# facebook/winterfell

Measured on NVIDIA H100. Metric: prover_ms, lower is better.
Workload: dtype u64

## Files before the change

### winterfell_b200/csrc/gl64.cuh

```cuda
#pragma once
#ifdef __CUDACC_RTC__
typedef unsigned long long uint64_t;
typedef unsigned int uint32_t;
typedef unsigned char uint8_t;
#else
#include <stdint.h>
#endif

#ifdef __CUDACC__
#define GL_HD __host__ __device__ __forceinline__
#else
#define GL_HD inline
#endif

typedef uint64_t u64;
typedef uint32_t u32;
typedef uint8_t u8;

#define GL_P 0xffffffff00000001ULL
#define GL_EPS 0xffffffffULL
#define GL_GENERATOR 7ULL
#define GL_TWO_ADIC_ROOT 7277203076849721926ULL

static inline u64 gl_add_host(u64 a, u64 b) {
    u64 r = a + b;
    if (r < a || r >= GL_P) r += GL_EPS;
    return r;
}
static inline u64 gl_sub_host(u64 a, u64 b) {
    u64 r = a - b;
    if (a < b) r -= GL_EPS;
    return r;
}
static inline u64 gl_reduce128_host(u64 lo, u64 hi) {
    u64 hh = hi >> 32, hl = hi & GL_EPS;
    u64 t = lo - hh;
    if (lo < hh) t -= GL_EPS;
    u64 m = (hl << 32) - hl;
    u64 r = t + m;
    if (r < m) r += GL_EPS;
    if (r >= GL_P) r -= GL_P;
    return r;
}

#if defined(__CUDACC__) && !defined(GL_LITERAL_EPS)
static __constant__ u32 GL_EPS_CONST = 0xffffffffu;
#define GL_EPS_OPERAND , "r"(GL_EPS_CONST)
#define GL_EPSM(n) "%" #n
#else
#define GL_EPS_OPERAND
#define GL_EPSM(n) "0xffffffff"
#endif
#ifdef __CUDA_ARCH__
__device__ __forceinline__ u64 gl_sub(u64 a, u64 b) {
    u64 r;
    asm("{\n\t"
        ".reg .u32 a0, a1, b0, b1, m;\n\t"
        "mov.b64 {a0, a1}, %1;\n\t"
        "mov.b64 {b0, b1}, %2;\n\t"
        "sub.cc.u32 a0, a0, b0;\n\t"
        "subc.cc.u32 a1, a1, b1;\n\t"
        "subc.u32 m, 0, 0;\n\t"
        "sub.cc.u32 a0, a0, m;\n\t"
        "subc.u32 a1, a1, 0;\n\t"
        "mov.b64 %0, {a0, a1};\n\t"
        "}"
        : "=l"(r)
        : "l"(a), "l"(b));
    return r;
}
__device__ __forceinline__ u64 gl_add(u64 a, u64 b) {
    u64 r;
    asm("{\n\t"
        ".reg .u32 a0, a1, b0, b1, m;\n\t"
        "mov.b64 {a0, a1}, %1;\n\t"
        "mov.b64 {b0, b1}, %2;\n\t"
        "sub.cc.u32 b0, 1, b0;\n\t"
        "subc.u32 b1, 0xffffffff, b1;\n\t"
        "sub.cc.u32 a0, a0, b0;\n\t"
        "subc.cc.u32 a1, a1, b1;\n\t"
        "subc.u32 m, 0, 0;\n\t"
        "sub.cc.u32 a0, a0, m;\n\t"
        "subc.u32 a1, a1, 0;\n\t"
        "mov.b64 %0, {a0, a1};\n\t"
        "}"
        : "=l"(r)
        : "l"(a), "l"(b));
    return r;
}
__device__ __forceinline__ void gl_butterfly(u64& a, u64& b) {
    u64 s, d;
    asm("{\n\t"
        ".reg .u32 a0, a1, b0, b1, n0, n1, s0, s1, m;\n\t"
        "mov.b64 {a0, a1}, %2;\n\t"
        "mov.b64 {b0, b1}, %3;\n\t"
        "sub.cc.u32 n0, 1, b0;\n\t"
        "subc.u32 n1, 0xffffffff, b1;\n\t"
        "sub.cc.u32 s0, a0, n0;\n\t"
        "subc.cc.u32 s1, a1, n1;\n\t"
        "subc.u32 m, 0, 0;\n\t"
        "sub.cc.u32 s0, s0, m;\n\t"
        "subc.u32 s1, s1, 0;\n\t"
        "mov.b64 %0, {s0, s1};\n\t"
        "sub.cc.u32 a0, a0, b0;\n\t"
        "subc.cc.u32 a1, a1, b1;\n\t"
        "subc.u32 m, 0, 0;\n\t"
        "sub.cc.u32 a0, a0, m;\n\t"
        "subc.u32 a1, a1, 0;\n\t"
        "mov.b64 %1, {a0, a1};\n\t"
        "}"
        : "=l"(s), "=l"(d)
        : "l"(a), "l"(b));
    a = s;
    b = d;
}
__device__ __forceinline__ u64 gl_canon(u64 r) {
    u64 o;
    asm("{\n\t"
        ".reg .u32 r0, r1, t0, t1, k;\n\t"
        "mov.b64 {r0, r1}, %1;\n\t"
        "add.cc.u32 t0, r0, 0xffffffff;\n\t"
        "addc.cc.u32 t1, r1, 0;\n\t"
        "addc.u32 k, 0, 0;\n\t"
        "sub.u32 r0, r0, k;\n\t"
        "add.u32 r1, r1, k;\n\t"
        "mov.b64 %0, {r0, r1};\n\t"
        "}"
        : "=l"(o)
        : "l"(r));
    return o;
}
__device__ __forceinline__ u64 gl_reduce128(u64 lo, u64 hi) {
    u64 r;
    asm("{\n\t"
        ".reg .u32 c0, c1, c2, c3, k, m, t0, t1;\n\t"
        "mov.b64 {c0, c1}, %1;\n\t"
        "mov.b64 {c2, c3}, %2;\n\t"
        "sub.cc.u32 c0, c0, c3;\n\t"
        "subc.cc.u32 c1, c1, 0;\n\t"
        "subc.u32 m, 0, 0;\n\t"
        "sub.cc.u32 c0, c0, m;\n\t"
        "subc.u32 c1, c1, 0;\n\t"
        "mad.lo.cc.u32 c0, c2, " GL_EPSM(3) ", c0;\n\t"
        "madc.hi.cc.u32 c1, c2, " GL_EPSM(3) ", c1;\n\t"
        "addc.u32 k, 0, 0;\n\t"
        "add.cc.u32 t0, c0, 0xffffffff;\n\t"
        "addc.cc.u32 t1, c1, 0;\n\t"
        "addc.u32 k, k, 0;\n\t"
        "mad.lo.cc.u32 c0, k, " GL_EPSM(3) ", c0;\n\t"
        "madc.hi.u32 c1, k, " GL_EPSM(3) ", c1;\n\t"
        "mov.b64 %0, {c0, c1};\n\t"
        "}"
        : "=l"(r)
        : "l"(lo), "l"(hi) GL_EPS_OPERAND);
    return r;
}
__device__ __forceinline__ u64 gl_mul(u64 a, u64 b) {
    u64 r;
    asm("{\n\t"
        ".reg .u32 a0, a1, b0, b1, c0, c1, c2, c3, o0, o1, o2, k, m, t0, t1;\n\t"
        "mov.b64 {a0, a1}, %1;\n\t"
        "mov.b64 {b0, b1}, %2;\n\t"
        "mul.lo.u32 c0, a0, b0;\n\t"
        "mul.hi.u32 c1, a0, b0;\n\t"
        "mul.lo.u32 c2, a1, b1;\n\t"
        "mul.hi.u32 c3, a1, b1;\n\t"
        "mul.lo.u32 o0, a0, b1;\n\t"
        "mul.hi.u32 o1, a0, b1;\n\t"
        "mad.lo.cc.u32 o0, a1, b0, o0;\n\t"
        "madc.hi.cc.u32 o1, a1, b0, o1;\n\t"
        "addc.u32 o2, 0, 0;\n\t"
        "add.cc.u32 c1, c1, o0;\n\t"
        "addc.cc.u32 c2, c2, o1;\n\t"
        "addc.u32 c3, c3, o2;\n\t"
        "sub.cc.u32 c0, c0, c3;\n\t"
        "subc.cc.u32 c1, c1, 0;\n\t"
        "subc.u32 m, 0, 0;\n\t"
        "sub.cc.u32 c0, c0, m;\n\t"
        "subc.u32 c1, c1, 0;\n\t"
        "mad.lo.cc.u32 c0, c2, " GL_EPSM(3) ", c0;\n\t"
        "madc.hi.cc.u32 c1, c2, " GL_EPSM(3) ", c1;\n\t"
        "addc.u32 k, 0, 0;\n\t"
        "add.cc.u32 t0, c0, 0xffffffff;\n\t"
        "addc.cc.u32 t1, c1, 0;\n\t"
        "addc.u32 k, k, 0;\n\t"
        "mad.lo.cc.u32 c0, k, " GL_EPSM(3) ", c0;\n\t"
        "madc.hi.u32 c1, k, " GL_EPSM(3) ", c1;\n\t"
        "mov.b64 %0, {c0, c1};\n\t"
        "}"
        : "=l"(r)
        : "l"(a), "l"(b) GL_EPS_OPERAND);
    return r;
}
__device__ __forceinline__ u64 gl_mul_weak(u64 a, u64 b) {
    u64 r;
    asm("{\n\t"
        ".reg .u32 a0, a1, b0, b1, c0, c1, c2, c3, o0, o1, o2, k, m;\n\t"
        "mov.b64 {a0, a1}, %1;\n\t"
        "mov.b64 {b0, b1}, %2;\n\t"
        "mul.lo.u32 c0, a0, b0;\n\t"
        "mul.hi.u32 c1, a0, b0;\n\t"
        "mul.lo.u32 c2, a1, b1;\n\t"
        "mul.hi.u32 c3, a1, b1;\n\t"
        "mul.lo.u32 o0, a0, b1;\n\t"
        "mul.hi.u32 o1, a0, b1;\n\t"
        "mad.lo.cc.u32 o0, a1, b0, o0;\n\t"
        "madc.hi.cc.u32 o1, a1, b0, o1;\n\t"
        "addc.u32 o2, 0, 0;\n\t"
        "add.cc.u32 c1, c1, o0;\n\t"
        "addc.cc.u32 c2, c2, o1;\n\t"
        "addc.u32 c3, c3, o2;\n\t"
        "sub.cc.u32 c0, c0, c3;\n\t"
        "subc.cc.u32 c1, c1, 0;\n\t"
        "subc.u32 m, 0, 0;\n\t"
        "sub.cc.u32 c0, c0, m;\n\t"
        "subc.u32 c1, c1, 0;\n\t"
        "mad.lo.cc.u32 c0, c2, " GL_EPSM(3) ", c0;\n\t"
        "madc.hi.cc.u32 c1, c2, " GL_EPSM(3) ", c1;\n\t"
        "addc.u32 k, 0, 0;\n\t"
        "mad.lo.cc.u32 c0, k, " GL_EPSM(3) ", c0;\n\t"
        "madc.hi.u32 c1, k, " GL_EPSM(3) ", c1;\n\t"
        "mov.b64 %0, {c0, c1};\n\t"
        "}"
        : "=l"(r)
        : "l"(a), "l"(b) GL_EPS_OPERAND);
    return r;
}
__device__ __forceinline__ u64 gl_sqr_weak(u64 a) {
    u64 r;
    asm("{\n\t"
        ".reg .u32 a0, a1, c0, c1, c2, c3, o0, o1, o2, k, m;\n\t"
        ".reg .u64 w;\n\t"
        "mov.b64 {a0, a1}, %1;\n\t"
        "mul.wide.u32 w, a0, a0;\n\t"
        "mov.b64 {c0, c1}, w;\n\t"
        "mul.wide.u32 w, a1, a1;\n\t"
        "mov.b64 {c2, c3}, w;\n\t"
        "mul.wide.u32 w, a0, a1;\n\t"
        "mov.b64 {o0, o1}, w;\n\t"
        "add.cc.u32 o0, o0, o0;\n\t"
        "addc.cc.u32 o1, o1, o1;\n\t"
        "addc.u32 o2, 0, 0;\n\t"
        "add.cc.u32 c1, c1, o0;\n\t"
        "addc.cc.u32 c2, c2, o1;\n\t"
        "addc.u32 c3, c3, o2;\n\t"
        "sub.cc.u32 c0, c0, c3;\n\t"
        "subc.cc.u32 c1, c1, 0;\n\t"
        "subc.u32 m, 0, 0;\n\t"
        "sub.cc.u32 c0, c0, m;\n\t"
        "subc.u32 c1, c1, 0;\n\t"
        "mad.lo.cc.u32 c0, c2, " GL_EPSM(2) ", c0;\n\t"
        "madc.hi.cc.u32 c1, c2, " GL_EPSM(2) ", c1;\n\t"
        "addc.u32 k, 0, 0;\n\t"
        "mad.lo.cc.u32 c0, k, " GL_EPSM(2) ", c0;\n\t"
        "madc.hi.u32 c1, k, " GL_EPSM(2) ", c1;\n\t"
        "mov.b64 %0, {c0, c1};\n\t"
        "}"
        : "=l"(r)
        : "l"(a) GL_EPS_OPERAND);
    return r;
}
template <int K>
__device__ __forceinline__ u64 gl_shl_dev(u64 x) {
    constexpr int R = K & 31;
    const u32 x0 = (u32)x, x1 = (u32)(x >> 32);
    const u32 y0 = x0 << R, y1 = R ? __funnelshift_l(x0, x1, R) : x1, y2 = R ? (x1 >> ((32 - R) & 31)) : 0;
    u64 o;
    if (K < 32) {
        asm("{\n\t"
            ".reg .u32 r0, r1, k, t0, t1;\n\t"
            "mad.lo.cc.u32 r0, %3, " GL_EPSM(4) ", %1;\n\t"
            "madc.hi.cc.u32 r1, %3, " GL_EPSM(4) ", %2;\n\t"
            "addc.u32 k, 0, 0;\n\t"
            "add.cc.u32 t0, r0, 0xffffffff;\n\t"
            "addc.cc.u32 t1, r1, 0;\n\t"
            "addc.u32 k, k, 0;\n\t"
            "mad.lo.cc.u32 r0, k, " GL_EPSM(4) ", r0;\n\t"
            "madc.hi.u32 r1, k, " GL_EPSM(4) ", r1;\n\t"
            "mov.b64 %0, {r0, r1};\n\t"
            "}" : "=l"(o) : "r"(y0), "r"(y1), "r"(y2) GL_EPS_OPERAND);
    } else if (K < 64) {
        asm("{\n\t"
            ".reg .u32 r0, r1, k, m, t0, t1;\n\t"
            "sub.cc.u32 r0, 0, %3;\n\t"
            "subc.cc.u32 r1, %1, 0;\n\t"
            "subc.u32 m, 0, 0;\n\t"
            "sub.cc.u32 r0, r0, m;\n\t"
            "subc.u32 r1, r1, 0;\n\t"
            "mad.lo.cc.u32 r0, %2, " GL_EPSM(4) ", r0;\n\t"
            "madc.hi.cc.u32 r1, %2, " GL_EPSM(4) ", r1;\n\t"
            "addc.u32 k, 0, 0;\n\t"
            "add.cc.u32 t0, r0, 0xffffffff;\n\t"
            "addc.cc.u32 t1, r1, 0;\n\t"
            "addc.u32 k, k, 0;\n\t"
            "mad.lo.cc.u32 r0, k, " GL_EPSM(4) ", r0;\n\t"
            "madc.hi.u32 r1, k, " GL_EPSM(4) ", r1;\n\t"
            "mov.b64 %0, {r0, r1};\n\t"
            "}" : "=l"(o) : "r"(y0), "r"(y1), "r"(y2) GL_EPS_OPERAND);
    } else {
        asm("{\n\t"
            ".reg .u32 m0, m1, b;\n\t"
            "mul.lo.u32 m0, %1, " GL_EPSM(4) ";\n\t"
            "mul.hi.u32 m1, %1, " GL_EPSM(4) ";\n\t"
            "sub.cc.u32 m0, m0, %2;\n\t"
            "subc.cc.u32 m1, m1, %3;\n\t"
            "subc.u32 b, 0, 0;\n\t"
            "sub.cc.u32 m0, m0, b;\n\t"
            "subc.u32 m1, m1, 0;\n\t"
            "mov.b64 %0, {m0, m1};\n\t"
            "}" : "=l"(o) : "r"(y0), "r"(y1), "r"(y2) GL_EPS_OPERAND);
    }
    return o;
}
#else
GL_HD u64 gl_add(u64 a, u64 b) { return gl_add_host(a, b); }
GL_HD u64 gl_sub(u64 a, u64 b) { return gl_sub_host(a, b); }
GL_HD u64 gl_reduce128(u64 lo, u64 hi) { return gl_reduce128_host(lo, hi); }
GL_HD u64 gl_mul(u64 a, u64 b) {
    unsigned __int128 x = (unsigned __int128)a * b;
    return gl_reduce128((u64)x, (u64)(x >> 64));
}
GL_HD u64 gl_mul_weak(u64 a, u64 b) { return gl_mul(a, b); }
GL_HD u64 gl_sqr_weak(u64 a) { return gl_mul(a, a); }
static inline void gl_butterfly(u64& a, u64& b) {
    u64 s = gl_add(a, b);
    b = gl_sub(a, b);
    a = s;
}
#endif
#ifdef __CUDACC__
struct GlAcc {
    u32 w0, w1, w2, w3, w4;
};
__device__ __forceinline__ GlAcc acc_zero() { return GlAcc{0, 0, 0, 0, 0}; }
__device__ __forceinline__ void acc_mad(GlAcc& a, u64 x, u64 y) {
    asm("{\n\t"
        ".reg .u32 x0, x1, y0, y1, m0, m1, m2;\n\t"
        "mov.b64 {x0, x1}, %5;\n\t"
        "mov.b64 {y0, y1}, %6;\n\t"
        "mul.lo.u32 m0, x0, y1;\n\t"
        "mul.hi.u32 m1, x0, y1;\n\t"
        "mad.lo.cc.u32 m0, x1, y0, m0;\n\t"
        "madc.hi.cc.u32 m1, x1, y0, m1;\n\t"
        "addc.u32 m2, 0, 0;\n\t"
        "mad.lo.cc.u32 %0, x0, y0, %0;\n\t"
        "madc.hi.cc.u32 %1, x0, y0, %1;\n\t"
        "madc.lo.cc.u32 %2, x1, y1, %2;\n\t"
        "madc.hi.cc.u32 %3, x1, y1, %3;\n\t"
        "addc.u32 %4, %4, 0;\n\t"
        "add.cc.u32 %1, %1, m0;\n\t"
        "addc.cc.u32 %2, %2, m1;\n\t"
        "addc.cc.u32 %3, %3, m2;\n\t"
        "addc.u32 %4, %4, 0;\n\t"
        "}"
        : "+r"(a.w0), "+r"(a.w1), "+r"(a.w2), "+r"(a.w3), "+r"(a.w4)
        : "l"(x), "l"(y));
}
__device__ __forceinline__ u64 acc_reduce(const GlAcc& a) {
    const u64 t = gl_reduce128((u64)a.w0 | ((u64)a.w1 << 32), (u64)a.w2 | ((u64)a.w3 << 32));
    return gl_sub(t, (u64)a.w4 << 32);
}
#endif
GL_HD u64 gl_neg(u64 a) { return a ? GL_P - a : 0; }
GL_HD u64 gl_dbl(u64 a) { return gl_add(a, a); }
GL_HD u64 gl_sqr(u64 a) { return gl_mul(a, a); }

template <int K>
GL_HD u64 gl_mul_2exp(u64 x) {
    if (K == 0) return x;
    if (K == 96) return gl_neg(x);
#ifdef __CUDA_ARCH__
    return gl_shl_dev<K>(x);
#else
    if (K < 64) return gl_reduce128(x << (K & 63), x >> ((64 - K) & 63));
    u64 yl = x << ((K - 64) & 63), yh = (K == 64) ? 0 : (x >> ((128 - K) & 63));
    u64 r = gl_reduce128(0, yl);
    return gl_sub(r, gl_reduce128(yh << 32, 0));
#endif
}

GL_HD u64 gl_pow(u64 a, u64 e) {
    u64 r = 1;
    while (e) {
        if (e & 1) r = gl_mul(r, a);
        a = gl_mul(a, a);
        e >>= 1;
    }
    return r;
}
GL_HD u64 gl_sqr_n(u64 a, int n) {
    for (int i = 0; i < n; i++) a = gl_sqr(a);
    return a;
}
GL_HD u64 gl_inv(u64 x) {
    u64 e2 = gl_mul(gl_sqr(x), x);
    u64 e4 = gl_mul(gl_sqr_n(e2, 2), e2);
    u64 e8 = gl_mul(gl_sqr_n(e4, 4), e4);
    u64 e16 = gl_mul(gl_sqr_n(e8, 8), e8);
    u64 e24 = gl_mul(gl_sqr_n(e16, 8), e8);
    u64 e28 = gl_mul(gl_sqr_n(e24, 4), e4);
    u64 e30 = gl_mul(gl_sqr_n(e28, 2), e2);
    u64 e31 = gl_mul(gl_sqr(e30), x);
    u64 a2 = gl_sqr(e31);
    u64 b = gl_mul(a2, x);
    return gl_mul(gl_sqr_n(a2, 32), b);
}
GL_HD u64 gl_root_of_unity(u32 log_n) { return gl_pow(GL_TWO_ADIC_ROOT, 1ULL << (32 - log_n)); }
GL_HD u64 gl_from_mont(u64 m) { return gl_mul(m, 18446744065119617025ULL); }
GL_HD u64 gl_to_mont(u64 x) { return gl_mul(x, GL_EPS); }

template <int D>
struct GlExt {
    u64 v[D];
};

template <int D>
GL_HD GlExt<D> ext_zero() {
    GlExt<D> r;
#pragma unroll
    for (int i = 0; i < D; i++) r.v[i] = 0;
    return r;
}
template <int D>
GL_HD GlExt<D> ext_from_base(u64 b) {
    GlExt<D> r = ext_zero<D>();
    r.v[0] = b;
    return r;
}
template <int D>
GL_HD GlExt<D> ext_add(const GlExt<D>& a, const GlExt<D>& b) {
    GlExt<D> r;
#pragma unroll
    for (int i = 0; i < D; i++) r.v[i] = gl_add(a.v[i], b.v[i]);
    return r;
}
template <int D>
GL_HD GlExt<D> ext_sub(const GlExt<D>& a, const GlExt<D>& b) {
    GlExt<D> r;
#pragma unroll
    for (int i = 0; i < D; i++) r.v[i] = gl_sub(a.v[i], b.v[i]);
    return r;
}
template <int D>
GL_HD GlExt<D> ext_mul_base(const GlExt<D>& a, u64 b) {
    GlExt<D> r;
#pragma unroll
    for (int i = 0; i < D; i++) r.v[i] = gl_mul(a.v[i], b);
    return r;
}
GL_HD GlExt<1> ext_mul(const GlExt<1>& a, const GlExt<1>& b) {
    GlExt<1> r;
    r.v[0] = gl_mul(a.v[0], b.v[0]);
    return r;
}
GL_HD GlExt<2> ext_mul(const GlExt<2>& a, const GlExt<2>& b) {
    GlExt<2> r;
    u64 a0b0 = gl_mul(a.v[0], b.v[0]);
    r.v[0] = gl_sub(a0b0, gl_dbl(gl_mul(a.v[1], b.v[1])));
    r.v[1] = gl_sub(gl_mul(gl_add(a.v[0], a.v[1]), gl_add(b.v[0], b.v[1])), a0b0);
    return r;
}
GL_HD GlExt<3> ext_mul(const GlExt<3>& a, const GlExt<3>& b) {
    GlExt<3> r;
    u64 a0b0 = gl_mul(a.v[0], b.v[0]), a1b1 = gl_mul(a.v[1], b.v[1]), a2b2 = gl_mul(a.v[2], b.v[2]);
    u64 s01 = gl_mul(gl_add(a.v[0], a.v[1]), gl_add(b.v[0], b.v[1]));
    u64 s02 = gl_mul(gl_add(a.v[0], a.v[2]), gl_add(b.v[0], b.v[2]));
    u64 s12 = gl_mul(gl_add(a.v[1], a.v[2]), gl_add(b.v[1], b.v[2]));
    u64 m = gl_sub(a0b0, a1b1);
    r.v[0] = gl_sub(gl_add(s12, m), a2b2);
    r.v[1] = gl_sub(gl_sub(gl_add(s01, s12), gl_dbl(a1b1)), a0b0);
    r.v[2] = gl_sub(s02, m);
    return r;
}
GL_HD GlExt<1> ext_frobenius(const GlExt<1>& x) { return x; }
GL_HD GlExt<2> ext_frobenius(const GlExt<2>& x) {
    GlExt<2> r;
    r.v[0] = gl_add(x.v[0], x.v[1]);
    r.v[1] = gl_neg(x.v[1]);
    return r;
}
GL_HD GlExt<3> ext_frobenius(const GlExt<3>& x) {
    GlExt<3> r;
    r.v[0] = gl_add(x.v[0], gl_add(gl_mul(10615703402128488253ULL, x.v[1]), gl_mul(6700183068485440220ULL, x.v[2])));
    r.v[1] = gl_add(gl_mul(10050274602728160328ULL, x.v[1]), gl_mul(14531223735771536287ULL, x.v[2]));
    r.v[2] = gl_add(gl_mul(11746561000929144102ULL, x.v[1]), gl_mul(8396469466686423992ULL, x.v[2]));
    return r;
}
GL_HD GlExt<1> ext_inv(const GlExt<1>& a) {
    GlExt<1> r;
    r.v[0] = gl_inv(a.v[0]);
    return r;
}
GL_HD GlExt<2> ext_inv(const GlExt<2>& a) {
    if ((a.v[0] | a.v[1]) == 0) return a;
    GlExt<2> num = ext_frobenius(a);
    GlExt<2> norm = ext_mul(a, num);
    return ext_mul_base(num, gl_inv(norm.v[0]));
}
GL_HD GlExt<3> ext_inv(const GlExt<3>& a) {
    if ((a.v[0] | a.v[1] | a.v[2]) == 0) return a;
    GlExt<3> c1 = ext_frobenius(a);
    GlExt<3> c2 = ext_frobenius(c1);
    GlExt<3> num = ext_mul(c1, c2);
    GlExt<3> norm = ext_mul(a, num);
    return ext_mul_base(num, gl_inv(norm.v[0]));
}
template <int D>
GL_HD GlExt<D> ext_pow(GlExt<D> a, u64 e) {
    GlExt<D> r = ext_from_base<D>(1);
    while (e) {
        if (e & 1) r = ext_mul(r, a);
        a = ext_mul(a, a);
        e >>= 1;
    }
    return r;
}
```

### winterfell_b200/csrc/minidft.cuh

```cuda
#pragma once
#include "gl64.cuh"

__device__ __forceinline__ void bf2(u64& a, u64& b) { gl_butterfly(a, b); }
template <int R>
__device__ __forceinline__ void mini_dft(u64* x);
template <>
__device__ __forceinline__ void mini_dft<1>(u64* x) { bf2(x[0], x[1]); }
template <>
__device__ __forceinline__ void mini_dft<2>(u64* x) {
    bf2(x[0], x[2]);
    bf2(x[1], x[3]);
    x[3] = gl_mul_2exp<48>(x[3]);
    bf2(x[0], x[1]);
    bf2(x[2], x[3]);
}
template <>
__device__ __forceinline__ void mini_dft<3>(u64* x);
template <>
__device__ __forceinline__ void mini_dft<3>(u64* x) {
    bf2(x[0], x[4]);
    bf2(x[1], x[5]);
    bf2(x[2], x[6]);
    bf2(x[3], x[7]);
    x[5] = gl_mul_2exp<24>(x[5]);
    x[6] = gl_mul_2exp<48>(x[6]);
    x[7] = gl_mul_2exp<72>(x[7]);
    mini_dft<2>(x);
    mini_dft<2>(x + 4);
}
template <>
__device__ __forceinline__ void mini_dft<4>(u64* x) {
    bf2(x[0], x[8]);
    bf2(x[1], x[9]);
    bf2(x[2], x[10]);
    bf2(x[3], x[11]);
    bf2(x[4], x[12]);
    bf2(x[5], x[13]);
    bf2(x[6], x[14]);
    bf2(x[7], x[15]);
    x[9] = gl_mul_2exp<12>(x[9]);
    x[10] = gl_mul_2exp<24>(x[10]);
    x[11] = gl_mul_2exp<36>(x[11]);
    x[12] = gl_mul_2exp<48>(x[12]);
    x[13] = gl_mul_2exp<60>(x[13]);
    x[14] = gl_mul_2exp<72>(x[14]);
    x[15] = gl_mul_2exp<84>(x[15]);
    mini_dft<3>(x);
    mini_dft<3>(x + 8);
}
template <>
__device__ __forceinline__ void mini_dft<5>(u64* x) {
#pragma unroll
    for (int q = 0; q < 16; q++) bf2(x[q], x[q + 16]);
    x[17] = gl_mul_2exp<6>(x[17]);
    x[18] = gl_mul_2exp<12>(x[18]);
    x[19] = gl_mul_2exp<18>(x[19]);
    x[20] = gl_mul_2exp<24>(x[20]);
    x[21] = gl_mul_2exp<30>(x[21]);
    x[22] = gl_mul_2exp<36>(x[22]);
    x[23] = gl_mul_2exp<42>(x[23]);
    x[24] = gl_mul_2exp<48>(x[24]);
    x[25] = gl_mul_2exp<54>(x[25]);
    x[26] = gl_mul_2exp<60>(x[26]);
    x[27] = gl_mul_2exp<66>(x[27]);
    x[28] = gl_mul_2exp<72>(x[28]);
    x[29] = gl_mul_2exp<78>(x[29]);
    x[30] = gl_mul_2exp<84>(x[30]);
    x[31] = gl_mul_2exp<90>(x[31]);
    mini_dft<4>(x);
    mini_dft<4>(x + 16);
}
__device__ __forceinline__ u32 brev(u32 v, int bits) { return __brev(v) >> (32 - bits); }

__device__ __forceinline__ u64 tw_lookup(const u64* tab, u32 e, u32 half) {
    u64 t = tab[e & (half - 1)];
    return (e & half) ? gl_neg(t) : t;
}
```

### winterfell_b200/csrc/ntt2.cu

```cuda
#include "minidft.cuh"
#include "ntt.cuh"

#ifndef NTT2_THREADS
#define NTT2_THREADS 256
#endif
#ifndef NTT2_MINB
#define NTT2_MINB 2
#endif
#define NTT2_TILE_ELEMS 8192

template <int LOGS>
struct Plan {
    static constexpr int rounds = LOGS >= 9 ? 3 : 2;
    static constexpr int r0 = (LOGS == 8) ? 4 : 3;
    static constexpr int r1 = (LOGS == 11 || LOGS == 8 || LOGS == 7) ? 4 : 3;
    static constexpr int r2 = LOGS >= 9 ? LOGS - r0 - r1 : 0;
    static_assert(LOGS >= 6 && LOGS <= 11, "plan covers 2^6 .. 2^11");
    static_assert(r0 + r1 + r2 == LOGS && (rounds == 2 || (r2 == 3 || r2 == 4)), "radices must add up");
    static constexpr int lanes = LOGS == 11 ? 4 : 8;
    static constexpr int tw0_entries = 1 << LOGS;
    static constexpr int tw1_entries = rounds == 3 ? (1 << (LOGS - r0)) : 0;
    static constexpr int tw_entries = tw0_entries + tw1_entries;
};
template <int LOGS> __host__ __device__ constexpr int plan_radix(int k) { return k == 0 ? Plan<LOGS>::r0 : (k == 1 ? Plan<LOGS>::r1 : Plan<LOGS>::r2); }
template <int LOGS> __host__ __device__ constexpr int plan_stage(int k) { return k == 0 ? 0 : (k == 1 ? Plan<LOGS>::r0 : Plan<LOGS>::r0 + Plan<LOGS>::r1); }

template <int LK>
__host__ __device__ constexpr u32 swz_const(u32 r) {
    u32 x = r >> LK, h = 0;
    while (x) { h ^= x & ((1u << LK) - 1); x >>= LK; }
    return h;
}
template <int LK>
__device__ __forceinline__ u32 swz_hash(u32 r) {
    if (LK == 1) return __popc(r >> 1) & 1;
    u32 x = r >> 2;
    x ^= x >> 4;
    x ^= x >> 8;
    x ^= x >> 2;
    return x & 3;
}
template <int LK>
__device__ __forceinline__ u32 prow(u32 r) { return r ^ swz_hash<LK>(r); }

__device__ __forceinline__ void bulk_init(u64* mbar, int tid) {
    if (tid == 0) {
        u32 mb = (u32)__cvta_generic_to_shared(mbar);
        asm volatile("mbarrier.init.shared::cta.b64 [%0], 1;" ::"r"(mb));
        asm volatile("fence.mbarrier_init.release.cluster;" ::: "memory");
    }
}
__device__ __forceinline__ void bulk_expect(u64* mbar, u32 bytes) {
    u32 mb = (u32)__cvta_generic_to_shared(mbar);
    asm volatile("mbarrier.arrive.expect_tx.shared::cta.b64 _, [%0], %1;" ::"r"(mb), "r"(bytes) : "memory");
}
__device__ __forceinline__ void bulk_copy(void* smem_dst, const void* gsrc, u32 bytes, u64* mbar) {
    u32 mb = (u32)__cvta_generic_to_shared(mbar), dst = (u32)__cvta_generic_to_shared(smem_dst);
    asm volatile("cp.async.bulk.shared::cluster.global.mbarrier::complete_tx::bytes [%0], [%1], %2, [%3];" ::"r"(dst), "l"(gsrc), "r"(bytes),
                 "r"(mb)
                 : "memory");
}
__device__ __forceinline__ void bulk_wait(u64* mbar) {
    u32 mb = (u32)__cvta_generic_to_shared(mbar), done = 0;
    while (!done)
        asm volatile("{\n\t.reg .pred p;\n\tmbarrier.try_wait.parity.shared::cta.b64 p, [%1], 0;\n\tselp.u32 %0, 1, 0, p;\n\t}" : "=r"(done) : "r"(mb) : "memory");
}

__device__ __forceinline__ void cp_async16(void* smem_dst, const void* gsrc, bool ok) {
    const u32 dst = (u32)__cvta_generic_to_shared(smem_dst);
    asm volatile("cp.async.cg.shared.global [%0], [%1], 16, %2;" ::"r"(dst), "l"(gsrc), "r"(ok ? 16 : 0) : "memory");
}
__device__ __forceinline__ void cp_async8(void* smem_dst, const void* gsrc, bool ok) {
    const u32 dst = (u32)__cvta_generic_to_shared(smem_dst);
    asm volatile("cp.async.ca.shared.global [%0], [%1], 8, %2;" ::"r"(dst), "l"(gsrc), "r"(ok ? 8 : 0) : "memory");
}
__device__ __forceinline__ void cp_async_commit() { asm volatile("cp.async.commit_group;" ::: "memory"); }
__device__ __forceinline__ void cp_async_wait_all() { asm volatile("cp.async.wait_group 0;" ::: "memory"); }

template <int LOGS, int K>
__device__ __forceinline__ void tile_round(u64* __restrict__ s, const u64* __restrict__ tw, const u64* __restrict__ pre, int tid) {
    constexpr int LANES = Plan<LOGS>::lanes, LK = LANES == 8 ? 1 : 2;
    constexpr int R = plan_radix<LOGS>(K), ST = plan_stage<LOGS>(K);
    constexpr int LOGSPAN = LOGS - ST - R;
    constexpr u32 SPAN = 1u << LOGSPAN;
    constexpr bool LAST = LOGSPAN == 0;
    constexpr u32 TASKS = (1u << LOGS) * LANES / 16;
    if (R == 4) {
        for (u32 task = tid; task < TASKS; task += NTT2_THREADS) {
            const u32 lane = task % LANES, bf = task / LANES;
            const u32 lo = bf & (SPAN - 1), base = ((bf >> LOGSPAN) << (LOGSPAN + 4)) + lo;
            const u32 hb = swz_hash<LK>(base);
            u64 x[16];
#pragma unroll
            for (int q = 0; q < 16; q++) {
                const u32 row = (base + ((u32)q << LOGSPAN)) ^ (hb ^ swz_const<LK>((u32)q << LOGSPAN));
                x[q] = s[row * LANES + lane];
            }
            if (K == 0 && pre) {
#pragma unroll
                for (int q = 0; q < 16; q++) x[q] = gl_mul(x[q], __ldg(pre + base + ((u32)q << LOGSPAN)));
            }
            mini_dft<4>(x);
            if (!LAST) {
                const ulonglong2* t2 = reinterpret_cast<const ulonglong2*>(tw + (size_t)lo * 16);
#pragma unroll
                for (int h = 0; h < 8; h++) {
                    const ulonglong2 w = t2[h];
                    if (h > 0) x[2 * h] = gl_mul(x[2 * h], w.x);
                    x[2 * h + 1] = gl_mul(x[2 * h + 1], w.y);
                }
            }
#pragma unroll
            for (int q = 0; q < 16; q++) {
                const u32 row = (base + ((u32)q << LOGSPAN)) ^ (hb ^ swz_const<LK>((u32)q << LOGSPAN));
                s[row * LANES + lane] = x[q];
            }
        }
    } else {
        constexpr int LP = LANES / 2;
        for (u32 task = tid; task < TASKS; task += NTT2_THREADS) {
            const u32 lp = task % LP, bf = task / LP;
            const u32 lo = bf & (SPAN - 1), base = ((bf >> LOGSPAN) << (LOGSPAN + 3)) + lo;
            const u32 hb = swz_hash<LK>(base);
            u64 xa[8], xb[8];
#pragma unroll
            for (int q = 0; q < 8; q++) {
                const u32 row = (base + ((u32)q << LOGSPAN)) ^ (hb ^ swz_const<LK>((u32)q << LOGSPAN));
                const ulonglong2 v = *reinterpret_cast<const ulonglong2*>(s + row * LANES + 2 * lp);
                xa[q] = v.x;
                xb[q] = v.y;
            }
            if (K == 0 && pre) {
#pragma unroll
                for (int q = 0; q < 8; q++) {
                    const u64 f = __ldg(pre + base + ((u32)q << LOGSPAN));
                    xa[q] = gl_mul(xa[q], f);
                    xb[q] = gl_mul(xb[q], f);
                }
            }
            mini_dft<3>(xa);
            mini_dft<3>(xb);
            if (!LAST) {
                const ulonglong2* t2 = reinterpret_cast<const ulonglong2*>(tw + (size_t)lo * 8);
#pragma unroll
                for (int h = 0; h < 4; h++) {
                    const ulonglong2 w = t2[h];
                    if (h > 0) { xa[2 * h] = gl_mul(xa[2 * h], w.x); xb[2 * h] = gl_mul(xb[2 * h], w.x); }
                    xa[2 * h + 1] = gl_mul(xa[2 * h + 1], w.y);
                    xb[2 * h + 1] = gl_mul(xb[2 * h + 1], w.y);
                }
            }
#pragma unroll
            for (int q = 0; q < 8; q++) {
                const u32 row = (base + ((u32)q << LOGSPAN)) ^ (hb ^ swz_const<LK>((u32)q << LOGSPAN));
                *reinterpret_cast<ulonglong2*>(s + row * LANES + 2 * lp) = make_ulonglong2(xa[q], xb[q]);
            }
        }
    }
}

template <int MODE, int LOGS>
__global__ void __launch_bounds__(NTT2_THREADS, NTT2_MINB) ntt2_pass_kernel(const NttPassParams p) {
    extern __shared__ __align__(16) u64 smem[];
    constexpr int LANES = Plan<LOGS>::lanes, LK = LANES == 8 ? 1 : 2, LP = LANES / 2;
    constexpr u32 S = 1u << LOGS;
    const int tid = threadIdx.x;
    const int W = p.W, logW = 31 - __clz(W);
    const int T = W >= LANES ? 1 : (LANES >> logW);
    const int chunks = W >= LANES ? W / LANES : 1;
    u64* s = smem;
    u64* rtw = s + (size_t)S * LANES;
    u64* ctw = rtw + Plan<LOGS>::tw_entries;
    u64* mbar = ctw + (p.has_post ? (size_t)S * T : 0);

    const bool ymap = p.y_in_out;
    const u32 tc = ymap ? blockIdx.y : blockIdx.x;
    const u32 tile = tc / chunks, q0 = (tc % chunks) * LANES;
    const u32 g = ymap ? blockIdx.z : blockIdx.y, b = ymap ? blockIdx.x : blockIdx.z;
    const u32 R = 1u << p.logR, C = 1u << p.logC;
    const u32 ncols = MODE == NTT_STRIDED ? C : R;

    {
        const u64* in = p.in + (size_t)g * p.in_seg_stride + (size_t)b * p.in_batch_stride;
        const u32 lp = tid % LP;
        const u32 l0 = 2 * lp;
        const u32 t0 = W >= LANES ? 0 : (l0 >> logW), t1 = W >= LANES ? 0 : ((l0 + 1) >> logW);
        const u32 w0 = W >= LANES ? q0 + l0 : (l0 & (W - 1)), w1 = W >= LANES ? q0 + l0 + 1 : ((l0 + 1) & (W - 1));
        const u32 c0 = tile * T + t0, c1 = tile * T + t1;
        const bool ok0 = c0 < ncols, ok1 = c1 < ncols;
        const bool yin = MODE == NTT_CONTIG && ymap;
        const u64 istride = MODE == NTT_STRIDED ? ((u64)W << p.logC) : (yin ? ((u64)p.out_row_mul << p.logR) * p.out_W : (u64)W);
        const u64* a0 = MODE == NTT_STRIDED ? in + (size_t)c0 * W + w0
                        : yin ? in + ((size_t)c0 * p.out_row_mul + (size_t)b * p.out_row_add) * p.out_W + p.out_col0 + w0
                              : in + (((size_t)c0 << p.logC) * W + w0);
        const u64* a1 = MODE == NTT_STRIDED ? in + (size_t)c1 * W + w1
                        : yin ? in + ((size_t)c1 * p.out_row_mul + (size_t)b * p.out_row_add) * p.out_W + p.out_col0 + w1
                              : in + (((size_t)c1 << p.logC) * W + w1);
        if (!ok0) a0 = p.in;
        if (!ok1) a1 = p.in;
        const u64 s0 = ok0 ? istride : 0, s1 = ok1 ? istride : 0;
        const bool vec = p.vec_in;
        constexpr u32 ROWS_PER_IT = NTT2_THREADS / LP;
#pragma unroll 4
        for (u32 i = tid / LP; i < S; i += ROWS_PER_IT) {
            u64* dst = s + prow<LK>(i) * LANES + l0;
            if (vec) {
                cp_async16(dst, a0 + i * s0, ok0);
            } else {
                cp_async8(dst, a0 + i * s0, ok0);
                cp_async8(dst + 1, a1 + i * s1, ok1);
            }
        }
        cp_async_commit();
    }

    bulk_init(mbar, tid);
    __syncthreads();
    if (tid == 0) {
        bulk_expect(mbar, Plan<LOGS>::tw_entries * 8);
        bulk_copy(rtw, p.sub_tw, Plan<LOGS>::tw_entries * 8, mbar);
    }

    if (p.has_post && T == 1) {
        const u32 M = 1u << p.logM, lo_mask = (1u << p.tw_split) - 1, c = tile;
        auto wpow = [&](u64 e64) {
            u32 e = (u32)(e64 & (M - 1));
            if (p.inverse && e) e = M - e;
            return gl_mul(p.tw_hi[e >> p.tw_split], p.tw_lo[e & lo_mask]);
        };
        u64 K = wpow((u64)(p.batch0 + b) * p.b_mul * c);
        if (p.ctab) K = gl_mul(K, p.ctab[c < ncols ? c : 0]);
        if (p.cconst != 1) K = gl_mul(K, p.cconst);
        const u64 step = wpow((u64)NTT2_THREADS * p.a_mul * c);
        u64 x = gl_mul(K, wpow((u64)tid * p.a_mul * c));
        for (u32 j = tid; j < S; j += NTT2_THREADS) {
            ctw[j] = x;
            x = gl_mul(x, step);
        }
    } else if (p.has_post) {
        const u32 M = 1u << p.logM, lo_mask = (1u << p.tw_split) - 1;
        for (u32 idx = tid; idx < S * (u32)T; idx += NTT2_THREADS) {
            const u32 j = idx / T, tt = idx % T, c = tile * T + tt;
            u64 e64 = ((u64)j * p.a_mul + (u64)(p.batch0 + b) * p.b_mul) * c;
            u32 e = (u32)(e64 & (M - 1));
            if (p.inverse && e) e = M - e;
            u64 x = gl_mul(p.tw_hi[e >> p.tw_split], p.tw_lo[e & lo_mask]);
            if (p.ctab) x = gl_mul(x, p.ctab[c < ncols ? c : 0]);
            if (p.cconst != 1) x = gl_mul(x, p.cconst);
            ctw[idx] = x;
        }
    }

    cp_async_wait_all();
    bulk_wait(mbar);
    __syncthreads();

    tile_round<LOGS, 0>(s, rtw, p.pre_tab ? p.pre_tab + (size_t)b * p.pre_batch_stride : nullptr, tid);
    __syncthreads();
    if (Plan<LOGS>::rounds == 3) {
        tile_round<LOGS, 1>(s, rtw + Plan<LOGS>::tw0_entries, nullptr, tid);
        __syncthreads();
        tile_round<LOGS, 2>(s, nullptr, nullptr, tid);
    } else {
        tile_round<LOGS, 1>(s, nullptr, nullptr, tid);
    }
    __syncthreads();

    u64* out = p.out + (size_t)g * p.out_seg_stride + (size_t)b * p.out_batch_stride;
    {
        const u32 lp = tid % LP, l0 = 2 * lp;
        const u32 t0 = W >= LANES ? 0 : (l0 >> logW), t1 = W >= LANES ? 0 : ((l0 + 1) >> logW);
        const u32 w0 = W >= LANES ? q0 + l0 : (l0 & (W - 1)), w1 = W >= LANES ? q0 + l0 + 1 : ((l0 + 1) & (W - 1));
        const u32 c0 = tile * T + t0, c1 = tile * T + t1;
        const bool ok0 = c0 < ncols, ok1 = c1 < ncols;
        u64 *o0, *o1, jstride;
        if (MODE == NTT_STRIDED && ymap) {
            o0 = out + (((size_t)c0 << p.logR) * p.out_row_mul + (size_t)b * p.out_row_add) * p.out_W + p.out_col0 + w0;
            o1 = out + (((size_t)c1 << p.logR) * p.out_row_mul + (size_t)b * p.out_row_add) * p.out_W + p.out_col0 + w1;
            jstride = (u64)p.out_row_mul * p.out_W;
        } else if (MODE == NTT_STRIDED) {
            o0 = out + (size_t)c0 * W + w0;
            o1 = out + (size_t)c1 * W + w1;
            jstride = (u64)W << p.logC;
        } else {
            o0 = out + ((size_t)c0 * p.out_row_mul + (size_t)b * p.out_row_add) * p.out_W + p.out_col0 + w0;
            o1 = out + ((size_t)c1 * p.out_row_mul + (size_t)b * p.out_row_add) * p.out_W + p.out_col0 + w1;
            jstride = ((u64)p.out_row_mul << p.logR) * p.out_W;
        }
        const bool post = p.has_post, scale = !p.has_post && p.cconst != 1, vec = p.vec_out;
        const u32 inv_mask = p.inverse ? (S - 1) : 0;
        constexpr u32 ROWS_PER_IT = NTT2_THREADS / LP;
#pragma unroll 4
        for (u32 j = tid / LP; j < S; j += ROWS_PER_IT) {
            const u32 jf = inv_mask ? ((S - j) & inv_mask) : j;
            const u32 r = __brev(jf) >> (32 - LOGS);
            ulonglong2 v = *reinterpret_cast<const ulonglong2*>(s + prow<LK>(r) * LANES + l0);
            if (post) {
                const u64 f0 = ctw[j * T + t0];
                v.x = gl_mul(v.x, f0);
                v.y = gl_mul(v.y, t1 == t0 ? f0 : ctw[j * T + t1]);
            } else if (scale) {
                v.x = gl_mul(v.x, p.cconst);
                v.y = gl_mul(v.y, p.cconst);
            }
            if (vec) {
                if (ok0) *reinterpret_cast<ulonglong2*>(o0 + (u64)j * jstride) = v;
            } else {
                if (ok0) o0[(u64)j * jstride] = v.x;
                if (ok1) o1[(u64)j * jstride] = v.y;
            }
        }
    }
}

template <int LOGS>
__global__ void ntt2_build_tw_kernel(u64* out, u64 w_s) {
    const u32 idx = blockIdx.x * blockDim.x + threadIdx.x;
    if (idx >= (u32)Plan<LOGS>::tw_entries) return;
    int k = idx < (u32)Plan<LOGS>::tw0_entries ? 0 : 1;
    const u32 li = k == 0 ? idx : idx - Plan<LOGS>::tw0_entries;
    const int r = plan_radix<LOGS>(k), st = plan_stage<LOGS>(k);
    const u32 lo = li >> r, qo = li & ((1u << r) - 1);
    const u32 e = (lo * (__brev(qo) >> (32 - r))) << st;
    out[idx] = gl_pow(w_s, e);
}

template <int LOGS>
static size_t smem_bytes_t(const NttPassParams& p) {
    const int lanes = Plan<LOGS>::lanes;
    const size_t S = (size_t)1 << LOGS, T = p.W >= lanes ? 1 : lanes / p.W;
    return (S * lanes + Plan<LOGS>::tw_entries + (p.has_post ? S * T : 0) + 2) * 8;
}
template <int MODE, int LOGS>
static cudaError_t launch_t(const NttPassParams& p, u32 n_segments, u32 n_batch, cudaStream_t st) {
    const int lanes = Plan<LOGS>::lanes;
    const u32 T = p.W >= lanes ? 1 : lanes / p.W, chunks = p.W >= lanes ? p.W / lanes : 1;
    const u32 ncols = MODE == NTT_STRIDED ? (1u << p.logC) : (1u << p.logR);
    const size_t smem = smem_bytes_t<LOGS>(p);
    const u32 tiles = ((ncols + T - 1) / T) * chunks;
    const dim3 grid = p.y_in_out ? dim3(n_batch, tiles, n_segments) : dim3(tiles, n_segments, n_batch);
    cudaError_t e = cudaFuncSetAttribute(ntt2_pass_kernel<MODE, LOGS>, cudaFuncAttributeMaxDynamicSharedMemorySize, (int)smem);
    if (e != cudaSuccess) return e;
    ntt2_pass_kernel<MODE, LOGS><<<grid, NTT2_THREADS, smem, st>>>(p);
    return cudaGetLastError();
}
template <int MODE>
static cudaError_t launch_m(const NttPassParams& p, u32 n_segments, u32 n_batch, cudaStream_t st) {
    switch (p.logS) {
        case 6: return launch_t<MODE, 6>(p, n_segments, n_batch, st);
        case 7: return launch_t<MODE, 7>(p, n_segments, n_batch, st);
        case 8: return launch_t<MODE, 8>(p, n_segments, n_batch, st);
        case 9: return launch_t<MODE, 9>(p, n_segments, n_batch, st);
        case 10: return launch_t<MODE, 10>(p, n_segments, n_batch, st);
        case 11: return launch_t<MODE, 11>(p, n_segments, n_batch, st);
    }
    return cudaErrorInvalidValue;
}
cudaError_t ntt2_launch_pass(int mode, const NttPassParams& p, u32 n_segments, u32 n_batch, cudaStream_t st) {
    return mode == NTT_STRIDED ? launch_m<NTT_STRIDED>(p, n_segments, n_batch, st) : launch_m<NTT_CONTIG>(p, n_segments, n_batch, st);
}
size_t ntt2_tw_entries(int logS) {
    switch (logS) {
        case 6: return Plan<6>::tw_entries; case 7: return Plan<7>::tw_entries; case 8: return Plan<8>::tw_entries;
        case 9: return Plan<9>::tw_entries; case 10: return Plan<10>::tw_entries; case 11: return Plan<11>::tw_entries;
    }
    return 0;
}
cudaError_t ntt2_build_tw(int logS, u64* d_out, cudaStream_t st) {
    const u64 w = gl_root_of_unity((u32)logS);
    const unsigned nb = (unsigned)((ntt2_tw_entries(logS) + 255) / 256);
    switch (logS) {
        case 6: ntt2_build_tw_kernel<6><<<nb, 256, 0, st>>>(d_out, w); break;
        case 7: ntt2_build_tw_kernel<7><<<nb, 256, 0, st>>>(d_out, w); break;
        case 8: ntt2_build_tw_kernel<8><<<nb, 256, 0, st>>>(d_out, w); break;
        case 9: ntt2_build_tw_kernel<9><<<nb, 256, 0, st>>>(d_out, w); break;
        case 10: ntt2_build_tw_kernel<10><<<nb, 256, 0, st>>>(d_out, w); break;
        case 11: ntt2_build_tw_kernel<11><<<nb, 256, 0, st>>>(d_out, w); break;
        default: return cudaErrorInvalidValue;
    }
    return cudaGetLastError();
}
```

Before: 92.55.

## Use lazy non-canonical reductions in NTT radix kernels with final canonicalization

Adds weak (non-canonical) Goldilocks add, sub, butterfly and shift routines, plus a carry-aware butterfly variant, and builds weak radix-4/8/16 mini-DFTs on them. The NTT pass kernels switch their butterflies, pre-multiplications and twiddle multiplies to these weak forms. Outputs are canonicalized at store time when no post-multiply or scale is applied. The aim is fewer reduction instructions per butterfly, at the cost of reasoning about intermediate value ranges across stages.

```diff
diff --git a/winterfell_b200/csrc/gl64.cuh b/winterfell_b200/csrc/gl64.cuh
--- a/winterfell_b200/csrc/gl64.cuh
+++ b/winterfell_b200/csrc/gl64.cuh
@@ -47,9 +47,14 @@
 static __constant__ u32 GL_EPS_CONST = 0xffffffffu;
 #define GL_EPS_OPERAND , "r"(GL_EPS_CONST)
 #define GL_EPSM(n) "%" #n
+static __constant__ u32 GL_ZERO_CONST = 0u;
+#define GL_ZERO_OPERAND , "r"(GL_ZERO_CONST)
+#define GL_CARRY(k, n) "madc.lo.u32 " k ", %" #n ", %" #n ", 0;\n\t"
 #else
 #define GL_EPS_OPERAND
 #define GL_EPSM(n) "0xffffffff"
+#define GL_ZERO_OPERAND
+#define GL_CARRY(k, n) "addc.u32 " k ", 0, 0;\n\t"
 #endif
 #ifdef __CUDA_ARCH__
 __device__ __forceinline__ u64 gl_sub(u64 a, u64 b) {
@@ -113,22 +118,6 @@
         : "l"(a), "l"(b));
     a = s;
     b = d;
-}
-__device__ __forceinline__ u64 gl_canon(u64 r) {
-    u64 o;
-    asm("{\n\t"
-        ".reg .u32 r0, r1, t0, t1, k;\n\t"
-        "mov.b64 {r0, r1}, %1;\n\t"
-        "add.cc.u32 t0, r0, 0xffffffff;\n\t"
-        "addc.cc.u32 t1, r1, 0;\n\t"
-        "addc.u32 k, 0, 0;\n\t"
-        "sub.u32 r0, r0, k;\n\t"
-        "add.u32 r1, r1, k;\n\t"
-        "mov.b64 %0, {r0, r1};\n\t"
-        "}"
-        : "=l"(o)
-        : "l"(r));
-    return o;
 }
 __device__ __forceinline__ u64 gl_reduce128(u64 lo, u64 hi) {
     u64 r;
@@ -379,6 +368,131 @@
 #endif
 }
 
+#ifdef __CUDACC__
+__device__ __forceinline__ u64 gl_canon(u64 r) {
+    u64 o;
+    asm("{\n\t"
+        ".reg .u32 r0, r1, t0, t1, k;\n\t"
+        "mov.b64 {r0, r1}, %1;\n\t"
+        "add.cc.u32 t0, r0, 0xffffffff;\n\t"
+        "addc.cc.u32 t1, r1, 0;\n\t"
+        "addc.u32 k, 0, 0;\n\t"
+        "sub.u32 r0, r0, k;\n\t"
+        "add.u32 r1, r1, k;\n\t"
+        "mov.b64 %0, {r0, r1};\n\t"
+        "}"
+        : "=l"(o)
+        : "l"(r));
+    return o;
+}
+
+__device__ __forceinline__ u64 gl_add_weak(u64 a, u64 b) {
+    u64 r;
+    asm("{\n\t"
+        ".reg .u32 a0, a1, b0, b1, k;\n\t"
+        "mov.b64 {a0, a1}, %1;\n\t"
+        "mov.b64 {b0, b1}, %2;\n\t"
+        "add.cc.u32 a0, a0, b0;\n\t"
+        "addc.cc.u32 a1, a1, b1;\n\t"
+        GL_CARRY("k", 4)
+        "mad.lo.cc.u32 a0, k, " GL_EPSM(3) ", a0;\n\t"
+        "madc.hi.cc.u32 a1, k, " GL_EPSM(3) ", a1;\n\t"
+        GL_CARRY("k", 4)
+        "mad.lo.cc.u32 a0, k, " GL_EPSM(3) ", a0;\n\t"
+        "madc.hi.u32 a1, k, " GL_EPSM(3) ", a1;\n\t"
+        "mov.b64 %0, {a0, a1};\n\t"
+        "}"
+        : "=l"(r)
+        : "l"(a), "l"(b) GL_EPS_OPERAND GL_ZERO_OPERAND);
+    return r;
+}
+__device__ __forceinline__ u64 gl_sub_weak(u64 a, u64 b) {
+    u64 r;
+    asm("{\n\t"
+        ".reg .u32 a0, a1, b0, b1, m;\n\t"
+        "mov.b64 {a0, a1}, %1;\n\t"
+        "mov.b64 {b0, b1}, %2;\n\t"
+        "sub.cc.u32 a0, a0, b0;\n\t"
+        "subc.cc.u32 a1, a1, b1;\n\t"
+        "subc.u32 m, 0, 0;\n\t"
+        "sub.cc.u32 a0, a0, m;\n\t"
+        "subc.cc.u32 a1, a1, 0;\n\t"
+        "subc.u32 m, 0, 0;\n\t"
+        "sub.cc.u32 a0, a0, m;\n\t"
+        "subc.u32 a1, a1, 0;\n\t"
+        "mov.b64 %0, {a0, a1};\n\t"
+        "}"
+        : "=l"(r)
+        : "l"(a), "l"(b));
+    return r;
+}
+__device__ __forceinline__ void gl_butterfly_weak(u64& a, u64& b) {
+    const u64 s = gl_add_weak(a, b);
+    b = gl_sub_weak(a, b);
+    a = s;
+}
+__device__ __forceinline__ void gl_butterfly_cb(u64& a, u64& b) {
+    u64 s, d;
+    asm("{\n\t"
+        ".reg .u32 a0, a1, b0, b1, s0, s1, k, m;\n\t"
+        "mov.b64 {a0, a1}, %2;\n\t"
+        "mov.b64 {b0, b1}, %3;\n\t"
+        "add.cc.u32 s0, a0, b0;\n\t"
+        "addc.cc.u32 s1, a1, b1;\n\t"
+        GL_CARRY("k", 5)
+        "mad.lo.cc.u32 s0, k, " GL_EPSM(4) ", s0;\n\t"
+        "madc.hi.u32 s1, k, " GL_EPSM(4) ", s1;\n\t"
+        "mov.b64 %0, {s0, s1};\n\t"
+        "sub.cc.u32 a0, a0, b0;\n\t"
+        "subc.cc.u32 a1, a1, b1;\n\t"
+        "subc.u32 m, 0, 0;\n\t"
+        "sub.cc.u32 a0, a0, m;\n\t"
+        "subc.u32 a1, a1, 0;\n\t"
+        "mov.b64 %1, {a0, a1};\n\t"
+        "}"
+        : "=l"(s), "=l"(d)
+        : "l"(a), "l"(b) GL_EPS_OPERAND GL_ZERO_OPERAND);
+    a = s;
+    b = d;
+}
+template <int K>
+__device__ __forceinline__ u64 gl_shl_weak(u64 x) {
+    static_assert(K > 0 && K < 96, "shift by 2^K for 0 < K < 96");
+    if (K >= 64) return gl_mul_2exp<K>(x);
+    constexpr int R = K & 31;
+    const u32 x0 = (u32)x, x1 = (u32)(x >> 32);
+    const u32 y0 = x0 << R, y1 = R ? __funnelshift_l(x0, x1, R) : x1, y2 = R ? (x1 >> ((32 - R) & 31)) : 0;
+    u64 o;
+    if (K < 32) {
+        asm("{\n\t"
+            ".reg .u32 r0, r1, k;\n\t"
+            "mad.lo.cc.u32 r0, %3, " GL_EPSM(4) ", %1;\n\t"
+            "madc.hi.cc.u32 r1, %3, " GL_EPSM(4) ", %2;\n\t"
+            GL_CARRY("k", 5)
+            "mad.lo.cc.u32 r0, k, " GL_EPSM(4) ", r0;\n\t"
+            "madc.hi.u32 r1, k, " GL_EPSM(4) ", r1;\n\t"
+            "mov.b64 %0, {r0, r1};\n\t"
+            "}" : "=l"(o) : "r"(y0), "r"(y1), "r"(y2) GL_EPS_OPERAND GL_ZERO_OPERAND);
+    } else {
+        asm("{\n\t"
+            ".reg .u32 r0, r1, k, m;\n\t"
+            "sub.cc.u32 r0, 0, %3;\n\t"
+            "subc.cc.u32 r1, %1, 0;\n\t"
+            "subc.u32 m, 0, 0;\n\t"
+            "sub.cc.u32 r0, r0, m;\n\t"
+            "subc.u32 r1, r1, 0;\n\t"
+            "mad.lo.cc.u32 r0, %2, " GL_EPSM(4) ", r0;\n\t"
+            "madc.hi.cc.u32 r1, %2, " GL_EPSM(4) ", r1;\n\t"
+            GL_CARRY("k", 5)
+            "mad.lo.cc.u32 r0, k, " GL_EPSM(4) ", r0;\n\t"
+            "madc.hi.u32 r1, k, " GL_EPSM(4) ", r1;\n\t"
+            "mov.b64 %0, {r0, r1};\n\t"
+            "}" : "=l"(o) : "r"(y0), "r"(y1), "r"(y2) GL_EPS_OPERAND GL_ZERO_OPERAND);
+    }
+    return o;
+}
+#endif
+
 GL_HD u64 gl_pow(u64 a, u64 e) {
     u64 r = 1;
     while (e) {
diff --git a/winterfell_b200/csrc/minidft.cuh b/winterfell_b200/csrc/minidft.cuh
--- a/winterfell_b200/csrc/minidft.cuh
+++ b/winterfell_b200/csrc/minidft.cuh
@@ -70,6 +70,39 @@
     mini_dft<4>(x);
     mini_dft<4>(x + 16);
 }
+
+template <int R, bool CB = false>
+__device__ __forceinline__ void mini_dft_weak(u64* x) {
+    static_assert(R >= 2 && R <= 4, "radix 4 .. 16");
+    constexpr int H = 1 << (R - 1);
+#pragma unroll
+    for (int q = 0; q < H; q++) {
+        if (CB) gl_butterfly_cb(x[q], x[q + H]);
+        else gl_butterfly_weak(x[q], x[q + H]);
+    }
+    if constexpr (R == 2) {
+        x[3] = gl_mul_2exp<48>(x[3]);
+        gl_butterfly_weak(x[0], x[1]);
+        gl_butterfly_cb(x[2], x[3]);
+    } else if constexpr (R == 3) {
+        x[5] = gl_shl_weak<24>(x[5]);
+        x[6] = gl_mul_2exp<48>(x[6]);
+        x[7] = gl_mul_2exp<72>(x[7]);
+        mini_dft_weak<2, false>(x);
+        mini_dft_weak<2, true>(x + 4);
+    } else {
+        x[9] = gl_shl_weak<12>(x[9]);
+        x[10] = gl_shl_weak<24>(x[10]);
+        x[11] = gl_shl_weak<36>(x[11]);
+        x[12] = gl_mul_2exp<48>(x[12]);
+        x[13] = gl_mul_2exp<60>(x[13]);
+        x[14] = gl_mul_2exp<72>(x[14]);
+        x[15] = gl_mul_2exp<84>(x[15]);
+        mini_dft_weak<3, false>(x);
+        mini_dft_weak<3, true>(x + 8);
+    }
+}
+
 __device__ __forceinline__ u32 brev(u32 v, int bits) { return __brev(v) >> (32 - bits); }
 
 __device__ __forceinline__ u64 tw_lookup(const u64* tab, u32 e, u32 half) {
diff --git a/winterfell_b200/csrc/ntt2.cu b/winterfell_b200/csrc/ntt2.cu
--- a/winterfell_b200/csrc/ntt2.cu
+++ b/winterfell_b200/csrc/ntt2.cu
@@ -98,16 +98,16 @@
             }
             if (K == 0 && pre) {
 #pragma unroll
-                for (int q = 0; q < 16; q++) x[q] = gl_mul(x[q], __ldg(pre + base + ((u32)q << LOGSPAN)));
-            }
-            mini_dft<4>(x);
+                for (int q = 0; q < 16; q++) x[q] = gl_mul_weak(x[q], __ldg(pre + base + ((u32)q << LOGSPAN)));
+            }
+            mini_dft_weak<4>(x);
             if (!LAST) {
                 const ulonglong2* t2 = reinterpret_cast<const ulonglong2*>(tw + (size_t)lo * 16);
 #pragma unroll
                 for (int h = 0; h < 8; h++) {
                     const ulonglong2 w = t2[h];
-                    if (h > 0) x[2 * h] = gl_mul(x[2 * h], w.x);
-                    x[2 * h + 1] = gl_mul(x[2 * h + 1], w.y);
+                    if (h > 0) x[2 * h] = gl_mul_weak(x[2 * h], w.x);
+                    x[2 * h + 1] = gl_mul_weak(x[2 * h + 1], w.y);
                 }
             }
 #pragma unroll
@@ -134,20 +134,20 @@
 #pragma unroll
                 for (int q = 0; q < 8; q++) {
                     const u64 f = __ldg(pre + base + ((u32)q << LOGSPAN));
-                    xa[q] = gl_mul(xa[q], f);
-                    xb[q] = gl_mul(xb[q], f);
+                    xa[q] = gl_mul_weak(xa[q], f);
+                    xb[q] = gl_mul_weak(xb[q], f);
                 }
             }
-            mini_dft<3>(xa);
-            mini_dft<3>(xb);
+            mini_dft_weak<3>(xa);
+            mini_dft_weak<3>(xb);
             if (!LAST) {
                 const ulonglong2* t2 = reinterpret_cast<const ulonglong2*>(tw + (size_t)lo * 8);
 #pragma unroll
                 for (int h = 0; h < 4; h++) {
                     const ulonglong2 w = t2[h];
-                    if (h > 0) { xa[2 * h] = gl_mul(xa[2 * h], w.x); xb[2 * h] = gl_mul(xb[2 * h], w.x); }
-                    xa[2 * h + 1] = gl_mul(xa[2 * h + 1], w.y);
-                    xb[2 * h + 1] = gl_mul(xb[2 * h + 1], w.y);
+                    if (h > 0) { xa[2 * h] = gl_mul_weak(xa[2 * h], w.x); xb[2 * h] = gl_mul_weak(xb[2 * h], w.x); }
+                    xa[2 * h + 1] = gl_mul_weak(xa[2 * h + 1], w.y);
+                    xb[2 * h + 1] = gl_mul_weak(xb[2 * h + 1], w.y);
                 }
             }
 #pragma unroll
@@ -302,6 +302,9 @@
             } else if (scale) {
                 v.x = gl_mul(v.x, p.cconst);
                 v.y = gl_mul(v.y, p.cconst);
+            } else {
+                v.x = gl_canon(v.x);
+                v.y = gl_canon(v.y);
             }
             if (vec) {
                 if (ok0) *reinterpret_cast<ulonglong2*>(o0 + (u64)j * jstride) = v;
```

Measured after the change: 90.93, median of 6. 1.02x faster.
